# nguyenduchuyiu/marl-delivery

Measured on AMD Instinct MI355X. Metric: agent-steps/sec (whole node), map1 5-agent 4096 envs, 1/2/4/8 MI355X, higher is better.
Workload: dtype int32+fp64

## Files before the change

### marl-delivery_amd/csrc/mdl_device.hpp

```cpp
#pragma once
#include <hip/hip_runtime.h>
#include <stdint.h>

#if !defined(MDL_PROFILING_BUILD) && \
    (defined(MDL_EXP_NOWAIT) || defined(MDL_EXP_NOTUPLES) || defined(MDL_EXP_NOLDS) || defined(MDL_ABLATE) || \
     defined(MDL_STAMPS))
#error "MDL_EXP_NOWAIT / MDL_EXP_NOTUPLES / MDL_EXP_NOLDS / MDL_ABLATE / MDL_STAMPS need -DMDL_PROFILING_BUILD"
#endif
#ifndef MDL_ABLATE
#define MDL_ABLATE 0
#endif

namespace mdl {

constexpr int WAVE = 64;
constexpr int MT_N = 624;
constexpr int MT_M = 397;
constexpr int MAX_MAPS = 8;
constexpr int PKG_PAD = 256;

enum : int { ST_NONE = 0, ST_WAITING = 1, ST_IN_TRANSIT = 2, ST_DELIVERED = 3 };
enum : int { MV_S = 0, MV_L = 1, MV_R = 2, MV_U = 3, MV_D = 4, MV_OTHER = 5 };
enum : int { SH_PICK = 0, SH_ONTIME, SH_LATE, SH_CLOSER, SH_WPICK, SH_WDROP, SH_STUCK, SH_IDLE, SH_AWAY };

struct MapDesc {
    int H, W, nfree;
    int grid_off;
    int free_off;
    int rank_off;
    float inv_hw;
    int bits_off;
    int mvc_off;
};

struct __align__(16) EnvScalars {
    int32_t t;
    uint32_t ctr;
    double total;
};
enum : uint32_t { RT_MOVE = 1u, RT_ONTIME = 2u, RT_LATE = 4u };

enum : uint32_t { PS_STATUS = 3u, PS_PRESENT = 4u, PS_TRANSIT = 8u, PS_SURVIVOR = 16u, PS_FLAGS = 31u };
constexpr int PS_RANK_SHIFT = 5;

constexpr uint32_t ORD_EPISODE = 0x400u;

struct DevParams {
    int E, A, P, T;
    double move_cost, delivery_reward, delay_reward;
    double cost_sum[9];
    float shaping[9];
    int stale;
    int obsT, MO, MP, MR, MPs;
    int n_maps;
    int key32_dsh;
    MapDesc maps[MAX_MAPS];
    const uint8_t* grids;
    const uint8_t* movevalid;
    const uint8_t* movevalid_cell;
    const uint32_t* gridbits;
    const uint16_t* free_cells;
    const uint16_t* rank;
    const uint8_t* env_map;
    uint32_t* rob;
    uint64_t* pkg;
    uint16_t* pstate;
    EnvScalars* es;
    uint32_t* mt;
    int32_t* mt_pos;
    uint64_t* trk;
    double* ep_total;
    int32_t* ep_len;
    const double* obs_recip;
    int obs_plane_words;
    int obs_small;
    int key7_dsh;
    double cost_fold[65];
};

__host__ __device__ __forceinline__ uint32_t rob_pack(int cell, int carry, uint32_t valid_mask ) {
    return (uint32_t)cell | ((uint32_t)carry << 16) | ((valid_mask & 0x1eu) << 26);
}
__host__ __device__ __forceinline__ int rob_cell(uint32_t w) { return (int)(w & 0xffffu); }
__host__ __device__ __forceinline__ int rob_carry(uint32_t w) { return (int)((w >> 16) & 0x7ffu); }
__host__ __device__ __forceinline__ uint32_t rob_valid(uint32_t w) { return (w >> 26) & 0x1eu; }

__device__ __forceinline__ int lane_id() { return (int)(threadIdx.x & 63); }
__device__ __forceinline__ int wave_id() { return __builtin_amdgcn_readfirstlane((int)(threadIdx.x >> 6)); }

__device__ __forceinline__ int xcd_slot(int b, int nb) { return (b & 7) * (nb >> 3) + min(b & 7, nb & 7) + (b >> 3); }
__device__ __forceinline__ int xcd_block() {
    return xcd_slot((int)blockIdx.x, (int)gridDim.x);
}

__device__ __forceinline__ void wave_sync() {
    __builtin_amdgcn_fence(__ATOMIC_RELEASE, "wavefront");
    __builtin_amdgcn_wave_barrier();
    __builtin_amdgcn_fence(__ATOMIC_ACQUIRE, "wavefront");
}

__device__ __forceinline__ uint64_t ballot(bool p) { return __ballot(p); }

#define GLOBAL __attribute__((address_space(1)))
typedef unsigned int u32x4 __attribute__((ext_vector_type(4)));

template <class T>
__device__ __forceinline__ void pin(T& v) { asm volatile("" : "+s"(v)); }

__device__ __forceinline__ int rdl(int v, int j) { return __builtin_amdgcn_readlane(v, j); }
__device__ __forceinline__ float rdlf(float v, int j) {
    return __int_as_float(__builtin_amdgcn_readlane(__float_as_int(v), j));
}
__device__ __forceinline__ int uni(int v) { return __builtin_amdgcn_readfirstlane(v); }

__device__ __forceinline__ uint32_t lmask(bool b) {
    uint32_t x = b ? ~0u : 0u;
    asm("" : "+v"(x));
    return x;
}
__device__ __forceinline__ uint32_t vbit(uint64_t m, int lane) { return 0u - (uint32_t)((m >> lane) & 1ull); }
__device__ __forceinline__ float fmask(uint32_t m, float a) { return __uint_as_float(m & __float_as_uint(a)); }
__device__ __forceinline__ float fpick(uint32_t m, float a, float b) {
    return __uint_as_float((m & __float_as_uint(a)) | (~m & __float_as_uint(b)));
}
__device__ __forceinline__ int ipick(uint32_t m, int a, int b) { return (int)((m & (uint32_t)a) | (~m & (uint32_t)b)); }

__device__ __forceinline__ int popc64(uint64_t m) { return __popcll(m); }
__device__ __forceinline__ int ffs64(uint64_t m) { return __ffsll((long long)m) - 1; }
__device__ __forceinline__ uint64_t lanemask_lt() {
    int l = lane_id();
    return l == 0 ? 0ull : (~0ull >> (64 - l));
}

__device__ __forceinline__ uint32_t wave_min_u32(uint32_t v) {
    const int id = (int)0xffffffff;
    uint32_t t;
    t = (uint32_t)__builtin_amdgcn_update_dpp(id, (int)v, 0x111, 0xf, 0xf, false); v = t < v ? t : v;
    t = (uint32_t)__builtin_amdgcn_update_dpp(id, (int)v, 0x112, 0xf, 0xf, false); v = t < v ? t : v;
    t = (uint32_t)__builtin_amdgcn_update_dpp(id, (int)v, 0x114, 0xf, 0xf, false); v = t < v ? t : v;
    t = (uint32_t)__builtin_amdgcn_update_dpp(id, (int)v, 0x118, 0xf, 0xf, false); v = t < v ? t : v;
    t = (uint32_t)__builtin_amdgcn_update_dpp(id, (int)v, 0x142, 0xa, 0xf, false); v = t < v ? t : v;
    t = (uint32_t)__builtin_amdgcn_update_dpp(id, (int)v, 0x143, 0xc, 0xf, false); v = t < v ? t : v;
    return (uint32_t)__builtin_amdgcn_readlane((int)v, 63);
}

__device__ __forceinline__ void wave_min_u32x2(uint32_t u, uint32_t v, uint32_t& mu, uint32_t& mv) {
    const int id = (int)0xffffffff;
    uint32_t a, b;
#define MDL_MIN2(ctl, rm)                                                                  \
    a = (uint32_t)__builtin_amdgcn_update_dpp(id, (int)u, ctl, rm, 0xf, false);            \
    b = (uint32_t)__builtin_amdgcn_update_dpp(id, (int)v, ctl, rm, 0xf, false);            \
    u = a < u ? a : u;                                                                     \
    v = b < v ? b : v;
    MDL_MIN2(0x111, 0xf)
    MDL_MIN2(0x112, 0xf)
    MDL_MIN2(0x114, 0xf)
    MDL_MIN2(0x118, 0xf)
    MDL_MIN2(0x142, 0xa)
    MDL_MIN2(0x143, 0xc)
#undef MDL_MIN2
    mu = (uint32_t)__builtin_amdgcn_readlane((int)u, 63);
    mv = (uint32_t)__builtin_amdgcn_readlane((int)v, 63);
}

__device__ __forceinline__ int wave_min8_lane(int a) { return ((a >> 1) << 4) | ((a & 1) << 3); }
__device__ __forceinline__ uint32_t wave_min8_u32(const uint32_t (&k)[8]) {
    uint32_t m[4], n[2];
#pragma unroll
    for (int i = 0; i < 4; i++) {
        const auto r = __builtin_amdgcn_permlane32_swap(k[i], k[i + 4], false, false);
        m[i] = r[0] < r[1] ? r[0] : r[1];
    }
#pragma unroll
    for (int i = 0; i < 2; i++) {
        const auto r = __builtin_amdgcn_permlane16_swap(m[i], m[i + 2], false, false);
        n[i] = r[0] < r[1] ? r[0] : r[1];
    }
    const bool hi = (lane_id() & 8) != 0;
    const uint32_t keep = hi ? n[1] : n[0], send = hi ? n[0] : n[1];
    const int id = (int)0xffffffff;
    uint32_t t = (uint32_t)__builtin_amdgcn_update_dpp(id, (int)send, 0x128, 0xf, 0xf, false);
    uint32_t v = t < keep ? t : keep;
    t = (uint32_t)__builtin_amdgcn_update_dpp(id, (int)v, 0x141, 0xf, 0xf, false);
    v = t < v ? t : v;
    t = (uint32_t)__builtin_amdgcn_update_dpp(id, (int)v, 0x4E, 0xf, 0xf, false);
    v = t < v ? t : v;
    t = (uint32_t)__builtin_amdgcn_update_dpp(id, (int)v, 0xB1, 0xf, 0xf, false);
    return t < v ? t : v;
}

__device__ __forceinline__ float qdiv_r(int a, double y) { return (float)((double)a * y); }

__device__ __forceinline__ float qdiv(int a, int b) { return (float)a / (float)b; }

__device__ __forceinline__ int fdivi(int i, int d, float inv) {
    int q = (int)((float)i * inv);
    int r = i - q * d;
    if (r < 0) q -= 1;
    else if (r >= d) q += 1;
    return q;
}

__device__ __forceinline__ int cell_r(int pc) { return pc & 255; }
__device__ __forceinline__ int cell_c(int pc) { return (pc >> 8) & 255; }
__device__ __forceinline__ int manhattan(int a, int b) {
    return abs(cell_r(a) - cell_r(b)) + abs(cell_c(a) - cell_c(b));
}
__device__ __forceinline__ int manhattan_sad(int a, int b) {
    return (int)__builtin_amdgcn_sad_u8((uint32_t)a, (uint32_t)b, 0u);
}

__device__ __forceinline__ int pk_start(uint64_t v) { return (int)(v & 0xffff); }
__device__ __forceinline__ int pk_target(uint64_t v) { return (int)((v >> 16) & 0xffff); }
__device__ __forceinline__ int pk_st(uint64_t v) { return (int)((v >> 32) & 0xffff); }
__device__ __forceinline__ int pk_dl(uint64_t v) { return (int)(v >> 48); }
__device__ __forceinline__ uint64_t pk_make(int start, int target, int st, int dl) {
    return (uint64_t)(uint32_t)start | ((uint64_t)(uint32_t)target << 16) | ((uint64_t)(uint32_t)st << 32) |
           ((uint64_t)(uint32_t)dl << 48);
}

__device__ __forceinline__ void decode_action(int a, int fmt, int& mv, int& op) {
    if (fmt == 0) {
        const int q = a / 5;
        const int m = a - 5 * q;
        mv = (0x30214 >> (4 * m)) & 0xf;
        op = q >= 3 ? 0 : q;
    } else {
        mv = a & 7;
        op = (a >> 3) & 3;
        if (mv > MV_OTHER) mv = MV_OTHER;
    }
}

__device__ inline void mt_twist(uint32_t* key) {
    const int lane = lane_id();
    for (int base = 0; base < MT_N; base += WAVE) {
        const int i = base + lane;
        uint32_t v = 0;
        if (i < MT_N) {
            const uint32_t y = (key[i] & 0x80000000u) | (key[i + 1 == MT_N ? 0 : i + 1] & 0x7fffffffu);
            const int k = i + MT_M < MT_N ? i + MT_M : i + MT_M - MT_N;
            v = key[k] ^ (y >> 1) ^ ((y & 1u) ? 0x9908b0dfu : 0u);
        }
        wave_sync();
        if (i < MT_N) key[i] = v;
        wave_sync();
    }
}

struct MTState {
    uint32_t* key;
    int pos;
};

__device__ inline uint32_t mt_next32(MTState& s) {
    if (s.pos == MT_N) {
        mt_twist(s.key);
        s.pos = 0;
    }
    uint32_t y = s.key[s.pos];
    s.pos++;
    y ^= (y >> 11);
    y ^= (y << 7) & 0x9d2c5680u;
    y ^= (y << 15) & 0xefc60000u;
    y ^= (y >> 18);
    return (uint32_t)uni((int)y);
}

__device__ inline int randint(MTState& s, int lo, int hi) {
    const uint32_t rng = (uint32_t)(hi - 1 - lo);
    if (rng == 0) return lo;
    uint32_t mask = rng;
    mask |= mask >> 1; mask |= mask >> 2; mask |= mask >> 4; mask |= mask >> 8; mask |= mask >> 16;
    uint32_t v;
    do {
        v = mt_next32(s) & mask;
    } while (v > rng);
    return lo + (int)v;
}

struct ResetOut {
    int robot_cell;
};

__device__ inline int reset_env(MTState& mt, const DevParams& p, const MapDesc& md, uint64_t* pk, uint8_t* pst,
                                uint64_t* scratch, uint16_t* taken) {
    const int lane = lane_id();
    const int A = p.A, P = p.P;
    const uint16_t* fl = p.free_cells + md.free_off;
    const int F = md.nfree;
    int my_cell = 0;
    int ntk = 0;
    for (int i = 0; i < A; i++) {
        const int k = randint(mt, 0, F - i);
        int idx = k;
        for (int q = 0; q < ntk; q++) {
            const int tq = taken[q];
            if (tq <= idx) idx++;
            else break;
        }
        if (lane == 0) {
            int q = ntk;
            while (q > 0 && taken[q - 1] > idx) {
                taken[q] = taken[q - 1];
                q--;
            }
            taken[q] = (uint16_t)idx;
        }
        ntk++;
        wave_sync();
        if (lane == i) my_cell = fl[idx];
    }
    const int N = md.H;
    const int lim = A < 20 ? A : 20;
    for (int i = 0; i < P; i++) {
        const int s_idx = randint(mt, 0, F);
        int t_idx;
        do {
            t_idx = randint(mt, 0, F);
        } while (t_idx == s_idx);
        const int to_dl = 10 + randint(mt, N / 2, 3 * N);
        const int st = (i <= lim) ? 0 : randint(mt, 1, p.T);
        if (lane == 0) scratch[i] = pk_make(s_idx, t_idx, st, st + to_dl);
    }
    wave_sync();
    for (int j = lane; j < P; j += WAVE) {
        const uint64_t v = scratch[j];
        scratch[j] = pk_make(fl[pk_start(v)], fl[pk_target(v)], pk_st(v), pk_dl(v));
    }
    wave_sync();
    for (int j0 = 0; j0 < P; j0 += WAVE) {
        const int j = j0 + lane;
        uint64_t v = 0;
        int sj = 0, rank = 0;
        if (j < P) {
            v = scratch[j];
            sj = pk_st(v);
        }
        for (int i = 0; i < P; i++) {
            const int si = pk_st(scratch[i]);
            rank += (si < sj) || (si == sj && i < j);
        }
        if (j < P) {
            pk[rank] = v;
        }
    }
    wave_sync();
    for (int j = lane; j < P; j += WAVE) pst[j] = pk_st(pk[j]) == 0 ? ST_WAITING : ST_NONE;
    wave_sync();
    return my_cell;
}

struct TrkFresh {
    static constexpr bool kIdIndexed = true;
    const uint64_t* pk;
    const uint8_t* ps;
    int n;
    __device__ int count() const { return n; }
    __device__ bool present(int j) const { const int s = ps[j] & PS_STATUS; return s == ST_WAITING || s == ST_IN_TRANSIT; }
    __device__ bool in_transit(int j) const { return (ps[j] & PS_STATUS) == ST_IN_TRANSIT; }
    __device__ uint64_t data(int j) const { return pk[j]; }
    __device__ int id(int j) const { return j + 1; }
    __device__ uint32_t order(int j) const { return (uint32_t)j; }
    __device__ int slot_of(int id) const { return (id >= 1 && id <= n && present(id - 1)) ? id - 1 : -1; }
};

struct TrkStale {
    static constexpr bool kIdIndexed = true;
    const uint8_t* ps;
    const uint64_t* td;
    const uint32_t* tq;
    int n;
    __device__ int count() const { return n; }
    __device__ bool present(int j) const { return (ps[j] & PS_PRESENT) != 0; }
    __device__ bool in_transit(int j) const { return (ps[j] & PS_TRANSIT) != 0; }
    __device__ uint64_t data(int j) const { return td[j]; }
    __device__ int id(int j) const { return j + 1; }
    __device__ uint32_t order(int j) const { return tq[j]; }
    __device__ int slot_of(int id) const { return (id >= 1 && id <= n && present(id - 1)) ? id - 1 : -1; }
};

struct TrkView {
    static constexpr bool kIdIndexed = false;
    const int32_t* ids;
    const uint8_t* flag;
    const uint64_t* pk;
    int n;
    __device__ int count() const { return n; }
    __device__ bool present(int j) const { return flag[j] & 1; }
    __device__ bool in_transit(int j) const { return (flag[j] & 2) != 0; }
    __device__ uint64_t data(int j) const { return pk[j]; }
    __device__ int id(int j) const { return ids[j]; }
    __device__ uint32_t order(int j) const { return (uint32_t)j; }
    __device__ int slot_of(int id) const {
        for (int j = 0; j < n; j++)
            if (ids[j] == id) return j;
        return -1;
    }
};

template <class Trk>
__device__ inline float shaped_agent(const Trk& trk, const float* C, bool active, int prev_cell, int prev_carry,
                                     int cur_cell, int cur_carry, int mv, int op, int t_prev, int t_cur) {
    float s = 0.0f;
    const int pslot = (active && prev_carry != 0) ? trk.slot_of(prev_carry) : -1;
    if (prev_carry == 0 && cur_carry != 0) {
        s = s + C[SH_PICK];
    } else if (prev_carry != 0 && cur_carry == 0) {
        if (pslot >= 0) {
            const uint64_t d = trk.data(pslot);
            if (cur_cell == pk_target(d)) s = s + ((t_cur <= pk_dl(d)) ? C[SH_ONTIME] : C[SH_LATE]);
        }
    }
    const bool moved = prev_cell != cur_cell;
    const bool need_can = active && op == 1 && prev_carry == 0 && cur_carry == 0;
    const bool need_near = active && moved && !(prev_carry != 0 && pslot >= 0);
    const bool need_idle = active && !moved && mv == MV_S && prev_carry == 0;
    bool can = false, idle = false;
    int best_d = 0x7fffffff;
    uint32_t best_o = 0xffffffffu;
    int best_cell = -1;
    if (__ballot(need_can || need_near || need_idle)) {
        const int n = trk.count();
        for (int j = 0; j < n; j++) {
            if (!trk.present(j) || trk.in_transit(j)) continue;
            const uint64_t d = trk.data(j);
            if (pk_st(d) > t_prev) continue;
            const int sc = pk_start(d);
            can |= sc == cur_cell;
            const int md = manhattan(prev_cell, sc);
            idle |= md <= 3;
            const uint32_t o = trk.order(j);
            if (md < best_d || (md == best_d && o < best_o)) {
                best_d = md;
                best_o = o;
                best_cell = sc;
            }
        }
    }
    if (op == 1) {
        if (prev_carry != 0) s = s + C[SH_WPICK];
        else if (cur_carry == 0 && !can) s = s + C[SH_WPICK];
    } else if (op == 2) {
        if (prev_carry == 0) s = s + C[SH_WDROP];
        else if (cur_carry != 0 && pslot >= 0 && cur_cell != pk_target(trk.data(pslot))) s = s + C[SH_WDROP];
    }
    if (mv != MV_S && !moved) s = s + C[SH_STUCK];
    int target = -1;
    if (prev_carry != 0 && pslot >= 0) target = pk_target(trk.data(pslot));
    else target = best_cell;
    if (target >= 0 && moved) {
        const int db = manhattan(prev_cell, target), da = manhattan(cur_cell, target);
        if (da < db) s = s + C[SH_CLOSER];
        else if (da > db) s = s + C[SH_AWAY];
    }
    if (!moved && mv == MV_S && prev_carry == 0 && idle) s = s + C[SH_IDLE];
    return active ? s : 0.0f;
}

template <int AU>
__device__ inline float np_sum_lanes8(float v, int n) {
    static_assert(AU >= 1 && AU <= 8, "np_sum_lanes8: 1 <= AU <= 8");
    float x[8];
#pragma unroll
    for (int i = 0; i < 8; i++) x[i] = i < AU ? rdlf(v, i) : 0.0f;
    float res;
    if (AU == 8 && n == 8) {
        res = ((x[0] + x[1]) + (x[2] + x[3])) + ((x[4] + x[5]) + (x[6] + x[7]));
    } else {
        res = 0.0f;
#pragma unroll
        for (int i = 0; i < (AU < 7 ? AU : 7); i++) res = res + x[i];
    }
    return 0.0f + res;
}

__device__ inline float np_sum_lanes(float v, int n) {
    float res;
    if (n < 8) {
        res = 0.0f;
        for (int i = 0; i < n; i++) res = res + rdlf(v, i);
    } else {
        float r0 = rdlf(v, 0), r1 = rdlf(v, 1), r2 = rdlf(v, 2), r3 = rdlf(v, 3);
        float r4 = rdlf(v, 4), r5 = rdlf(v, 5), r6 = rdlf(v, 6), r7 = rdlf(v, 7);
        int i;
        for (i = 8; i < n - (n % 8); i += 8) {
            r0 = r0 + rdlf(v, i + 0); r1 = r1 + rdlf(v, i + 1); r2 = r2 + rdlf(v, i + 2); r3 = r3 + rdlf(v, i + 3);
            r4 = r4 + rdlf(v, i + 4); r5 = r5 + rdlf(v, i + 5); r6 = r6 + rdlf(v, i + 6); r7 = r7 + rdlf(v, i + 7);
        }
        res = ((r0 + r1) + (r2 + r3)) + ((r4 + r5) + (r6 + r7));
        for (; i < n; i++) res = res + rdlf(v, i);
    }
    return 0.0f + res;
}

template <int AU>
__device__ inline float np_sum_lanes_dpp(float v) {
    static_assert(AU >= 1 && AU <= 7, "np_sum_lanes_dpp: 1 <= AU <= 7");
    float t = v;
#pragma unroll
    for (int i = 1; i < AU; i++) {
        const float prev = __int_as_float(__builtin_amdgcn_update_dpp(0, __float_as_int(t), 0x111, 0xf, 0xf, true));
        t = v + prev;
    }
    return rdlf(t, AU - 1);
}

template <int CTL>
__device__ __forceinline__ float dppf(float x) {
    return __int_as_float(__builtin_amdgcn_update_dpp(0, __float_as_int(x), CTL, 0xf, 0xf, true));
}
__device__ inline float np_sum16_dpp(float v) {
    const float r = v + dppf<0x128>(v);
    const float s = r + dppf<0xB1>(r);
    const float c = s + dppf<0x4E>(s);
    const float d = c + dppf<0x124>(c);
    return 0.0f + rdlf(d, 0);
}

template <int AU>
__device__ inline float np_sum_step(float v, int n) {
    if constexpr (AU > 0 && AU <= 7) return np_sum_lanes_dpp<AU>(v);
    else if constexpr (AU == 16) return np_sum16_dpp(v);
    else if constexpr (AU == 8) return np_sum_lanes8<AU>(v, n);
    else return np_sum_lanes(v, n);
}

}
```

### marl-delivery_amd/csrc/mdl_kernels.hip

```cpp
#include <cstring>
#include <type_traits>

#include "mdl_kernels.hpp"
#include "mdl_features.hpp"
#include "mdl_obs_small.hpp"
#include "mdl_altfeat.hpp"


namespace mdl {

#ifdef MDL_STAMPS
__device__ uint64_t g_stamps[65536 * 16];
#define STAMP(k)                                      \
    do {                                              \
        __builtin_amdgcn_sched_barrier(0);            \
        stamp_[k] = __builtin_amdgcn_s_memtime();     \
        __builtin_amdgcn_sched_barrier(0);            \
    } while (0)
#else
#define STAMP(k) \
    do {         \
    } while (0)
#endif

__host__ __device__ inline int stage_floats(int A, int na, int MO, int MPc, int MR, int MPsc) {
    const int dc = actor_compact_dim(A, MO, MPc);
    const int a = actor_group(na, dc) * dc, cr = critic_compact_dim(A, MR, MPsc);
    return a > cr ? a : cr;
}

struct ResetLds {
    uint64_t* pk;
    uint64_t* scratch;
    uint32_t* mt;
    uint16_t* taken;
    uint8_t* pst;
};

__host__ __device__ constexpr size_t reset_lds_bytes(int P) {
    return align16(8 * (size_t)P) * 2 + align16(4 * MT_N) + align16(2 * 64) + align16((size_t)P);
}

__device__ inline ResetLds reset_carve(unsigned char* b, int P) {
    ResetLds L;
    size_t o = 0;
    L.pk = (uint64_t*)(b + o); o += align16(8 * (size_t)P);
    L.scratch = (uint64_t*)(b + o); o += align16(8 * (size_t)P);
    L.mt = (uint32_t*)(b + o); o += align16(4 * MT_N);
    L.taken = (uint16_t*)(b + o); o += align16(2 * 64);
    L.pst = b + o;
    return L;
}

__device__ inline void load_mt(const DevParams& p, int e, uint32_t* key) {
    const uint32_t* g = p.mt + (size_t)e * MT_N;
    for (int i = lane_id(); i < MT_N; i += WAVE) key[i] = g[i];
    wave_sync();
}

__device__ inline void store_mt(const DevParams& p, int e, const uint32_t* key, int pos) {
    uint32_t* g = p.mt + (size_t)e * MT_N;
    for (int i = lane_id(); i < MT_N; i += WAVE) g[i] = key[i];
    if (lane_id() == 0) p.mt_pos[e] = pos;
}

__device__ inline int do_reset(const DevParams& p, int e, const MapDesc& md, ResetLds& L, bool seeded_in_lds) {
    if (!seeded_in_lds) load_mt(p, e, L.mt);
    MTState ms{L.mt, seeded_in_lds ? MT_N : p.mt_pos[e]};
    const int cell = reset_env(ms, p, md, L.pk, L.pst, L.scratch, L.taken);
    store_mt(p, e, L.mt, ms.pos);
    return cell;
}

template <int NCH, int AU = 0>
__device__ inline void tracker_update_regs(uint32_t (&ps)[NCH], uint64_t (&td)[NCH], bool (&dirty)[NCH],
                                           const uint64_t (&pk)[NCH], int P, int A, int carry, int t) {
    const int lane = lane_id();
#pragma unroll
    for (int c = 0; c < NCH; c++) {
        const int j = c * WAVE + lane;
        const bool ins = (j < P) & (pk_st(pk[c]) == t) & !(ps[c] & PS_PRESENT);
        ps[c] = ins ? ((ps[c] & PS_STATUS) | PS_PRESENT) : ps[c];
        td[c] = ins ? pk[c] : td[c];
        dirty[c] = dirty[c] || ins;
    }
#pragma unroll
    for (int c = 0; c < NCH; c++) {
        const int id = c * WAVE + lane + 1;
        bool carried = false;
        if constexpr (AU > 0) {
            uint32_t ci[AU], mn = 0xffffffffu;
#pragma unroll
            for (int i = 0; i < AU; i++) ci[i] = (uint32_t)rdl(carry, i);
            __builtin_amdgcn_sched_barrier(0);
#pragma unroll
            for (int i = 0; i < AU; i++) mn = min(mn, ci[i] ^ (uint32_t)id);
            carried = mn == 0u;
        } else {
            for (int i = 0; i < A; i++) carried |= rdl(carry, i) == id;
        }
        const uint32_t upd = carried ? (ps[c] | PS_TRANSIT) : (ps[c] & PS_TRANSIT) ? (ps[c] & PS_STATUS) : ps[c];
        ps[c] = (ps[c] & PS_PRESENT) ? upd : ps[c];
    }
}

template <int NCH>
__device__ inline void tracker_update_bits(uint32_t (&ps)[NCH], uint64_t (&td)[NCH], bool (&dirty)[NCH],
                                           const uint64_t (&pk)[NCH], int P, int t, uint32_t carried_bits) {
    const int lane = lane_id();
#pragma unroll
    for (int c = 0; c < NCH; c++) {
        const int j = c * WAVE + lane;
        const bool ins = (j < P) & (pk_st(pk[c]) == t) & !(ps[c] & PS_PRESENT);
        ps[c] = ins ? ((ps[c] & PS_STATUS) | PS_PRESENT) : ps[c];
        td[c] = ins ? pk[c] : td[c];
        dirty[c] = dirty[c] || ins;
        const bool carried = (carried_bits >> c) & 1u;
        const uint32_t upd = carried ? (ps[c] | PS_TRANSIT) : (ps[c] & PS_TRANSIT) ? (ps[c] & PS_STATUS) : ps[c];
        ps[c] = (ps[c] & PS_PRESENT) ? upd : ps[c];
    }
}

template <int NCH>
__device__ inline void survivors_at_reset(uint32_t (&ps)[NCH], uint32_t (&tq)[NCH], int P) {
    const int lane = lane_id();
    uint32_t rk[NCH];
#pragma unroll
    for (int c = 0; c < NCH; c++) rk[c] = 0;
#pragma unroll
    for (int c2 = 0; c2 < NCH; c2++) {
        uint64_t m = ballot(c2 * WAVE + lane < P && (ps[c2] & PS_PRESENT));
        while (m) {
            const uint32_t ki = (uint32_t)rdl((int)tq[c2], ffs64(m));
            m &= m - 1;
#pragma unroll
            for (int c = 0; c < NCH; c++) rk[c] += ki < tq[c] ? 1u : 0u;
        }
    }
#pragma unroll
    for (int c = 0; c < NCH; c++) {
        if (c * WAVE + lane < P && (ps[c] & PS_PRESENT)) {
            tq[c] = rk[c];
            ps[c] = (ps[c] & PS_FLAGS) | PS_SURVIVOR | (rk[c] << PS_RANK_SHIFT);
        } else {
            ps[c] &= PS_STATUS;
        }
    }
}

__global__ __launch_bounds__(256) void k_seed(DevParams p, const uint32_t* __restrict__ seeds, int wpb,
                                              int lds_stride) {
    extern __shared__ __align__(16) unsigned char smem[];
    const int wave = wave_id();
    const int lane = lane_id();
    const int e = blockIdx.x * wpb + wave;
    if (wave >= wpb || e >= p.E) return;
    ResetLds L = reset_carve(smem + (size_t)wave * lds_stride, p.P);
    const MapDesc md = p.maps[p.env_map ? p.env_map[e] : 0];
    if (lane == 0) {
        uint32_t s = seeds[e];
        for (int i = 0; i < MT_N; i++) {
            L.mt[i] = s;
            s = 1812433253u * (s ^ (s >> 30)) + (uint32_t)(i + 1);
        }
    }
    wave_sync();
    const int cell = do_reset(p, e, md, L, true);
    if (lane < p.A)
        p.rob[(size_t)e * p.A + lane] = rob_pack(cell, 0, p.movevalid[md.grid_off + cell_r(cell) * md.W + cell_c(cell)]);
    for (int j = lane; j < p.P; j += WAVE) {
        const size_t g = (size_t)e * p.P + j;
        p.pkg[g] = L.pk[j];
        p.pstate[g] = L.pst[j];
    }
    if (lane == 0) {
        EnvScalars s;
        s.t = 0;
        s.ctr = 0;
        s.total = 0.0;
        p.es[e] = s;
        p.ep_total[e] = 0.0;
        p.ep_len[e] = 0;
    }
}

template <int NCH>
__global__ __launch_bounds__(256) void k_reset(DevParams p, const int* __restrict__ env_ids, int n, int wpb,
                                               int lds_stride) {
    extern __shared__ __align__(16) unsigned char smem[];
    const int wave = wave_id();
    const int lane = lane_id();
    const int w = xcd_block() * wpb + wave;
    if (wave >= wpb || w >= n) return;
    const int e = env_ids ? env_ids[w] : w;
    if ((unsigned)e >= (unsigned)p.E) return;
    const int A = p.A, P = p.P;
    ResetLds L = reset_carve(smem + (size_t)wave * lds_stride, P);
    const MapDesc md = p.maps[p.env_map ? p.env_map[e] : 0];
    uint32_t ps[NCH], tq[NCH];
#pragma unroll
    for (int c = 0; c < NCH; c++) {
        const int j = c * WAVE + lane;
        ps[c] = j < P ? p.pstate[(size_t)e * P + j] : 0u;
        tq[c] = (p.stale && (ps[c] & PS_SURVIVOR)) ? ps[c] >> PS_RANK_SHIFT : ORD_EPISODE + (uint32_t)j;
    }
    const int cell = do_reset(p, e, md, L, false);
    uint64_t pk[NCH], td[NCH];
    bool dirty[NCH];
    if (p.stale) survivors_at_reset<NCH>(ps, tq, P);
#pragma unroll
    for (int c = 0; c < NCH; c++) {
        const int j = c * WAVE + lane;
        pk[c] = j < P ? L.pk[j] : 0;
        ps[c] = (j < P ? L.pst[j] : 0u) | (p.stale ? (ps[c] & ~PS_STATUS) : 0u);
        td[c] = pk[c];
        dirty[c] = false;
    }
    if (p.stale) tracker_update_regs<NCH>(ps, td, dirty, pk, P, A, 0, 0);
    if (lane < A)
        p.rob[(size_t)e * A + lane] = rob_pack(cell, 0, p.movevalid[md.grid_off + cell_r(cell) * md.W + cell_c(cell)]);
#pragma unroll
    for (int c = 0; c < NCH; c++) {
        const int j = c * WAVE + lane;
        if (j < P) {
            const size_t g = (size_t)e * P + j;
            p.pkg[g] = pk[c];
            p.pstate[g] = (uint16_t)ps[c];
            if (dirty[c]) p.trk[g] = td[c];
        }
    }
    if (lane == 0) {
        EnvScalars s;
        s.t = 0;
        s.ctr = 0;
        s.total = 0.0;
        p.es[e] = s;
    }
}

__global__ __launch_bounds__(256) void k_tracker_clear(DevParams p, const int* __restrict__ env_ids, int n) {
    const int wave = wave_id();
    const int w = blockIdx.x * 4 + wave;
    if (w >= n) return;
    const int e = env_ids ? env_ids[w] : w;
    if ((unsigned)e >= (unsigned)p.E) return;
    for (int j = lane_id(); j < p.P; j += WAVE) {
        const size_t g = (size_t)e * p.P + j;
        p.pstate[g] &= (uint16_t)PS_STATUS;
    }
    if (lane_id() == 0) p.es[e].ctr = 0;
}

#define MDL_STEP_LB 256
template <int NCH, bool FUSED>
constexpr int step_wpe() { return (NCH <= 2 && !FUSED) ? 8 : 1; }
#define MDL_STEP_ATTR(NCH, FUSED) __attribute__((amdgpu_waves_per_eu(step_wpe<NCH, FUSED>())))
struct StepArgs {
    DevParams p;
    const uint8_t* actions;
    const int* env_ids;
    double* r_out;
    float* sh_out;
    uint8_t* done_out;
    int fmt, n, auto_reset, wpb, lds_stride, K;
};
typedef __attribute__((address_space(4))) const StepArgs* KargPtr;
static_assert(sizeof(StepArgs) + 256 <= 4096, "the step's kernel arguments stay inside the 4 KiB kernarg segment");

struct StepKarg {
    const uint32_t* rob;
    const uint64_t* pkg;
    const uint16_t* pst;
    const u32x4* es;
    const uint64_t* trk;
    const uint8_t* act;
    uint32_t ap, nw;
    StepArgs args;
};
constexpr uint32_t NW_IDS = 1u << 29, NW_MAP = 1u << 30;
constexpr uint32_t NW_SMALLMAP = 1u << 31;
constexpr int AP_NB_SHIFT = 18;
inline uint32_t pack_ap(int A, int P, int nblocks) {
    const uint32_t nb = nblocks < (1 << (32 - AP_NB_SHIFT)) ? (uint32_t)nblocks : 0u;
    return (uint32_t)A | ((uint32_t)P << 7) | (nb << AP_NB_SHIFT);
}

struct ObsArgs {
    float* amap;
    float* avec;
    float* cmap;
    float* cvec;
};

struct EpiArgs {
    uint8_t* active;
    uint8_t* filled;
};
typedef __attribute__((address_space(4))) const EpiArgs* EpiKargPtr;
constexpr size_t EPI_KARG_OFF = sizeof(StepArgs) + sizeof(ObsArgs);
static_assert(sizeof(StepArgs) % 8 == 0 && sizeof(ObsArgs) % 8 == 0, "EpiArgs starts where ObsArgs ends");

__device__ __forceinline__ void publish_tail(const Publish& pb) {
    __atomic_thread_fence(__ATOMIC_RELEASE);
    if (!pb.ctr) {
        if (lane_id() == 0) __hip_atomic_store(pb.seq, pb.value, __ATOMIC_RELAXED, __HIP_MEMORY_SCOPE_SYSTEM);
        return;
    }
    if (lane_id() == 0) {
        const unsigned waves = pb.expect ? pb.expect : gridDim.x * (blockDim.x / WAVE);
        if (atomicAdd(pb.ctr, 1u) - pb.base == waves - 1u) {
            __atomic_thread_fence(__ATOMIC_ACQ_REL);
            __hip_atomic_store(pb.seq, pb.value, __ATOMIC_RELEASE, __HIP_MEMORY_SCOPE_SYSTEM);
        }
    }
}

constexpr int MAIL_INLINE_CODES = 256;
struct MailArgs {
    MailRows m;
    Publish pb;
    uint8_t codes[MAIL_INLINE_CODES];
};

#include "mdl_step_common.hpp"

__host__ __device__ constexpr uint64_t move_lt_lanes(int k) {
    uint64_t m = 0;
    for (int l = 0; l < 64; l++)
        if (((l >> 4) << 2) + k < (l & 15)) m |= 1ull << l;
    return m;
}

template <bool STALE, int NCH, bool FUSED, int AU, bool OBS, bool MAIL = false, bool EPI = false>
__device__ __forceinline__ void step_body(const uint32_t* __restrict__ rob_pre, const uint64_t* __restrict__ pkg_pre,
                                          const uint16_t* __restrict__ pst_pre, const u32x4* __restrict__ es_pre,
                                          const uint64_t* __restrict__ trk_pre, const uint8_t* __restrict__ act_pre,
                                          uint32_t ap, uint32_t nw, const StepArgs& args, const ObsArgs& oa,
                                          const MailArgs* ma = nullptr) {
    static_assert(!OBS || (NCH == 1 && !FUSED && AU > 0 && AU <= 8), "fused observations: P <= 64, A <= 8");
    static_assert(!EPI || (OBS && !MAIL), "the episode form is the fused step + observation launch's");
    extern __shared__ __align__(16) unsigned char smem[];
    const DevParams& p = args.p;
#ifdef MDL_STAMPS
    uint64_t stamp_[16];
#endif
    STAMP(0);
    const int A = (int)(ap & 0x7fu), P = (int)((ap >> 7) & 0x7ffu);
    const int n_ = (int)(nw & 0xffffffu), wpb_ = (int)((nw >> 24) & 31u);
    GLOBAL const uint32_t* robp = (GLOBAL const uint32_t*)rob_pre;
    GLOBAL const uint64_t* pkgp = (GLOBAL const uint64_t*)pkg_pre;
    GLOBAL const uint16_t* pstp = (GLOBAL const uint16_t*)pst_pre;
    GLOBAL const u32x4* esp = (GLOBAL const u32x4*)es_pre;
    GLOBAL const uint64_t* trkp = (GLOBAL const uint64_t*)trk_pre;
    GLOBAL const uint8_t* actp = (GLOBAL const uint8_t*)act_pre;
    STAMP(1);

    const int wave = wave_id();
    const int lane = lane_id();
    const int nbp = (int)(ap >> AP_NB_SHIFT);
    const int w = (nbp ? xcd_slot((int)blockIdx.x, nbp) : (int)blockIdx.x) * wpb_ + wave;
    if (wave >= wpb_ || w >= n_) return;
    int e = w;
    if (nw & NW_IDS) {
        e = uni(((GLOBAL const int*)args.env_ids)[w]);
        if ((unsigned)e >= (unsigned)args.p.E) return;
    }
    if constexpr (EPI) {
        KargPtr ka = (KargPtr)((__attribute__((address_space(4))) const char*)
                                   __builtin_amdgcn_kernarg_segment_ptr() + offsetof(StepKarg, args));
        asm volatile("" : "+s"(ka));
        EpiKargPtr ke = (EpiKargPtr)((__attribute__((address_space(4))) const char*)ka + EPI_KARG_OFF);
        if (!uni((int)((GLOBAL const uint8_t*)ke->active)[w])) {
            if (lane == 0) {
// ... 1744 lines not shown
```

Measured before the change: 4.956 billion.

## Batch MT tempering per wave window and use ballot-based reset sampling

Reworks the per-environment reset path. The Mersenne Twister now tempers a 64-word window in parallel across lanes and reads values via lane shuffles instead of serial LDS reads. Sampling without replacement uses ballot/popcount instead of a lane-0 sorted LDS list, and package records are built in registers and written in batches of 64. The rank sort now uses cross-lane reads instead of LDS, and the key is written back only when a twist happened. Each of these removes serial LDS traffic and wave syncs in reset, at the cost of more register state and more complex RNG bookkeeping.

```diff
diff --git a/marl-delivery_amd/csrc/mdl_device.hpp b/marl-delivery_amd/csrc/mdl_device.hpp
--- a/marl-delivery_amd/csrc/mdl_device.hpp
+++ b/marl-delivery_amd/csrc/mdl_device.hpp
@@ -251,27 +251,47 @@
 struct MTState {
     uint32_t* key;
     int pos;
-};
-
-__device__ inline uint32_t mt_next32(MTState& s) {
-    if (s.pos == MT_N) {
-        mt_twist(s.key);
-        s.pos = 0;
-    }
-    uint32_t y = s.key[s.pos];
-    s.pos++;
+    int wbase;
+    int wend;
+    uint32_t win;
+    bool twisted;
+};
+
+__device__ __forceinline__ void mt_refill(MTState& s, int base) {
+    const int i = base + lane_id();
+    uint32_t y = s.key[i < MT_N ? i : MT_N - 1];
     y ^= (y >> 11);
     y ^= (y << 7) & 0x9d2c5680u;
     y ^= (y << 15) & 0xefc60000u;
     y ^= (y >> 18);
-    return (uint32_t)uni((int)y);
-}
-
-__device__ inline int randint(MTState& s, int lo, int hi) {
-    const uint32_t rng = (uint32_t)(hi - 1 - lo);
-    if (rng == 0) return lo;
-    uint32_t mask = rng;
-    mask |= mask >> 1; mask |= mask >> 2; mask |= mask >> 4; mask |= mask >> 8; mask |= mask >> 16;
+    s.win = y;
+    s.wbase = base;
+    s.wend = base + WAVE < MT_N ? base + WAVE : MT_N;
+}
+
+__device__ __forceinline__ MTState mt_begin(uint32_t* key, int pos) { return MTState{key, pos, pos, pos, 0u, false}; }
+
+__device__ __forceinline__ void mt_drop_window(MTState& s) { s.wend = s.pos; }
+
+__device__ __forceinline__ uint32_t mt_next32(MTState& s) {
+    if (s.pos == s.wend) {
+        if (s.pos == MT_N) {
+            mt_twist(s.key);
+            s.twisted = true;
+            s.pos = 0;
+        }
+        mt_refill(s, s.pos);
+    }
+    const uint32_t y = (uint32_t)rdl((int)s.win, s.pos - s.wbase);
+    s.pos++;
+    return y;
+}
+
+__device__ __forceinline__ uint32_t rng_mask(uint32_t rng) { return rng ? 0xffffffffu >> __clz((int)rng) : 0u; }
+
+template <bool NONZERO = false>
+__device__ __forceinline__ int randint_m(MTState& s, int lo, uint32_t rng, uint32_t mask) {
+    if (!NONZERO && rng == 0) return lo;
     uint32_t v;
     do {
         v = mt_next32(s) & mask;
@@ -279,67 +299,69 @@
     return lo + (int)v;
 }
 
-struct ResetOut {
-    int robot_cell;
-};
+__device__ __forceinline__ int randint(MTState& s, int lo, int hi) {
+    const uint32_t rng = (uint32_t)(hi - 1 - lo);
+    return randint_m(s, lo, rng, rng_mask(rng));
+}
 
 __device__ inline int reset_env(MTState& mt, const DevParams& p, const MapDesc& md, uint64_t* pk, uint8_t* pst,
-                                uint64_t* scratch, uint16_t* taken) {
+                                uint64_t* scratch) {
     const int lane = lane_id();
     const int A = p.A, P = p.P;
     const uint16_t* fl = p.free_cells + md.free_off;
     const int F = md.nfree;
-    int my_cell = 0;
-    int ntk = 0;
+    int tk = 0x7fffffff;
     for (int i = 0; i < A; i++) {
         const int k = randint(mt, 0, F - i);
         int idx = k;
-        for (int q = 0; q < ntk; q++) {
-            const int tq = taken[q];
-            if (tq <= idx) idx++;
-            else break;
-        }
-        if (lane == 0) {
-            int q = ntk;
-            while (q > 0 && taken[q - 1] > idx) {
-                taken[q] = taken[q - 1];
-                q--;
-            }
-            taken[q] = (uint16_t)idx;
-        }
-        ntk++;
-        wave_sync();
-        if (lane == i) my_cell = fl[idx];
-    }
+        for (;;) {
+            const int nx = k + popc64(ballot(tk <= idx));
+            if (nx == idx) break;
+            idx = nx;
+        }
+        tk = lane == i ? idx : tk;
+    }
+    const int my_cell = lane < A ? (int)fl[tk] : 0;
     const int N = md.H;
     const int lim = A < 20 ? A : 20;
+    const uint32_t rng_f = (uint32_t)(F - 1), mask_f = rng_mask(rng_f);
+    const uint32_t rng_d = (uint32_t)(3 * N - 1 - N / 2), mask_d = rng_mask(rng_d);
+    const uint32_t rng_s = (uint32_t)(p.T - 2), mask_s = rng_mask(rng_s);
+    int rc = 0, rt = 0;
     for (int i = 0; i < P; i++) {
-        const int s_idx = randint(mt, 0, F);
+        const int s_idx = randint_m(mt, 0, rng_f, mask_f);
         int t_idx;
         do {
-            t_idx = randint(mt, 0, F);
+            t_idx = randint_m(mt, 0, rng_f, mask_f);
         } while (t_idx == s_idx);
-        const int to_dl = 10 + randint(mt, N / 2, 3 * N);
-        const int st = (i <= lim) ? 0 : randint(mt, 1, p.T);
-        if (lane == 0) scratch[i] = pk_make(s_idx, t_idx, st, st + to_dl);
-    }
-    wave_sync();
-    for (int j = lane; j < P; j += WAVE) {
-        const uint64_t v = scratch[j];
-        scratch[j] = pk_make(fl[pk_start(v)], fl[pk_target(v)], pk_st(v), pk_dl(v));
+        const int to_dl = 10 + randint_m<true>(mt, N / 2, rng_d, mask_d);
+        const int st = (i <= lim) ? 0 : randint_m(mt, 1, rng_s, mask_s);
+        const bool mine = lane == (i & 63);
+        rc = mine ? (s_idx | (t_idx << 16)) : rc;
+        rt = mine ? (st | ((st + to_dl) << 16)) : rt;
+        if ((i & 63) == 63 || i == P - 1) {
+            const int j = (i & ~63) + lane;
+            mt_drop_window(mt);
+            if (j <= i) scratch[j] = pk_make(fl[rc & 0xffff], fl[(uint32_t)rc >> 16], rt & 0xffff, (uint32_t)rt >> 16);
+        }
     }
     wave_sync();
     for (int j0 = 0; j0 < P; j0 += WAVE) {
         const int j = j0 + lane;
         uint64_t v = 0;
-        int sj = 0, rank = 0;
+        uint32_t kj = 0, rank = 0;
         if (j < P) {
             v = scratch[j];
-            sj = pk_st(v);
-        }
-        for (int i = 0; i < P; i++) {
-            const int si = pk_st(scratch[i]);
-            rank += (si < sj) || (si == sj && i < j);
+            kj = ((uint32_t)pk_st(v) << 10) | (uint32_t)j;
+        }
+        for (int i0 = 0; i0 < P; i0 += WAVE) {
+            const int il = i0 + lane;
+            const uint32_t ki = il < P ? ((uint32_t)pk_st(scratch[il]) << 10) | (uint32_t)il : 0xffffffffu;
+            const int n = uni(P - i0 < WAVE ? P - i0 : WAVE);
+            for (int i = 0; i < n; i += 4) {
+#pragma unroll
+                for (int u = 0; u < 4; u++) rank += (uint32_t)rdl((int)ki, i + u) < kj ? 1u : 0u;
+            }
         }
         if (j < P) {
             pk[rank] = v;
diff --git a/marl-delivery_amd/csrc/mdl_kernels.hip b/marl-delivery_amd/csrc/mdl_kernels.hip
--- a/marl-delivery_amd/csrc/mdl_kernels.hip
+++ b/marl-delivery_amd/csrc/mdl_kernels.hip
@@ -54,21 +54,37 @@
 
 __device__ inline void load_mt(const DevParams& p, int e, uint32_t* key) {
     const uint32_t* g = p.mt + (size_t)e * MT_N;
-    for (int i = lane_id(); i < MT_N; i += WAVE) key[i] = g[i];
+    const int lane = lane_id();
+#pragma unroll
+    for (int b = 0; b < 2; b++) {
+        uint32_t w[5];
+#pragma unroll
+        for (int k = 0; k < 5; k++) {
+            const int i = (b * 5 + k) * WAVE + lane;
+            w[k] = i < MT_N ? g[i] : 0u;
+        }
+#pragma unroll
+        for (int k = 0; k < 5; k++) {
+            const int i = (b * 5 + k) * WAVE + lane;
+            if (i < MT_N) key[i] = w[k];
+        }
+    }
     wave_sync();
 }
 
-__device__ inline void store_mt(const DevParams& p, int e, const uint32_t* key, int pos) {
-    uint32_t* g = p.mt + (size_t)e * MT_N;
-    for (int i = lane_id(); i < MT_N; i += WAVE) g[i] = key[i];
+__device__ inline void store_mt(const DevParams& p, int e, const uint32_t* key, int pos, bool key_changed) {
+    if (key_changed) {
+        uint32_t* g = p.mt + (size_t)e * MT_N;
+        for (int i = lane_id(); i < MT_N; i += WAVE) g[i] = key[i];
+    }
     if (lane_id() == 0) p.mt_pos[e] = pos;
 }
 
 __device__ inline int do_reset(const DevParams& p, int e, const MapDesc& md, ResetLds& L, bool seeded_in_lds) {
     if (!seeded_in_lds) load_mt(p, e, L.mt);
-    MTState ms{L.mt, seeded_in_lds ? MT_N : p.mt_pos[e]};
-    const int cell = reset_env(ms, p, md, L.pk, L.pst, L.scratch, L.taken);
-    store_mt(p, e, L.mt, ms.pos);
+    MTState ms = mt_begin(L.mt, seeded_in_lds ? MT_N : uni(p.mt_pos[e]));
+    const int cell = reset_env(ms, p, md, L.pk, L.pst, L.scratch);
+    store_mt(p, e, L.mt, ms.pos, seeded_in_lds || ms.twisted);
     return cell;
 }
 
```

New measurement: 4.995 billion (median of 6 runs). About the same (+0.8%).
